# HUSRCF/JaTSR-Just-audio-transformer-super-solution

Hardware: AMD Instinct MI355X
Metric: DiT latent-frames/sec (B=28,C=1024,T=512, 50-step CFG) (higher is better)
Workload: dtype bf16; 1 GPU; v3mod2 DiT 50-step CFG=3.0 flow-matching sampling, hipGraph, B=28/GPU C=1024 T=512; B_per_gpu=28, global_batch=28, T=512, C=1024, euler_steps=50, weights=recipe (random-init, non-zero adaLN/final), parallelism=replicas x1, no collective in the loop, rccl_ranks=1

## Files before the change

### include/jat_hip.h

```cpp
#ifndef JAT_HIP_H
#define JAT_HIP_H

#include <stddef.h>
#include <stdint.h>

#ifdef __cplusplus
extern "C" {
#endif

#define JAT_OK 0
#define JAT_E_INVALID (-1)
#define JAT_E_HIP (-2)
#define JAT_E_STATE (-3)
#define JAT_E_SEQLEN (-4)

#define JAT_NORM_RMS_W 0
#define JAT_NORM_LN_NOAFFINE 1

typedef struct jat_model jat_model;
typedef struct jat_sampler jat_sampler;

typedef struct jat_config {
  int32_t input_channels;
  int32_t cond_channels;
// ... 73 lines not shown
                      float max_grad_norm, float loss_scale, int32_t step, float* grad_norm_out, void* stream);

int jat_k_norm_modulate(const float* x, const float* w, const float* shift, const float* scale,
                        int64_t mod_bstride, uint16_t* y_bf16, int32_t M, int32_t D, int32_t rows_per_batch,
                        int32_t norm_mode, void* stream);
int jat_k_gemm(const uint16_t* A, const uint16_t* W, const float* bias, void* C, int32_t M, int32_t N,
               int32_t K, int32_t epilogue, const float* gate, int64_t gate_bstride, int32_t rows_per_batch,
               int32_t variant, void* stream);
int jat_k_gemm_fold(const uint16_t* A, const uint16_t* W, const float* bias, void* C, int32_t M, int32_t N, int32_t K,
                    int32_t epilogue, const float* gate, int64_t gate_bstride, int32_t rows_per_batch, uint16_t* hi,
                    uint16_t* lo, float* part_out, const float* part_in, int32_t part_in_np, int32_t variant, void* stream);
int jat_k_gemm_splitk(const uint16_t* A, const uint16_t* W, float* parts, int32_t M, int32_t N, int32_t K, int32_t ksplit,
                      int32_t variant, void* stream);
int jat_k_qkv_attn(const uint16_t* A, const uint16_t* Wg, const float* bias, uint16_t* out, int32_t M, int32_t Hkv, int32_t K,
                   const float* rope_inv_freq, const float* part_in, int32_t part_in_np, void* stream);
int jat_k_gemm_wave_n(int32_t variant);
int jat_k_weight_grad(const uint16_t* dY, const uint16_t* X, float* dW, float* db, int32_t tokens, int32_t out, int32_t in,
                      int32_t ksplit, void* work, size_t work_bytes, void* stream);
int jat_k_attention(const uint16_t* q, const uint16_t* k, const uint16_t* vt, uint16_t* o, int32_t B,
                    int32_t N, int32_t Hq, int32_t Hkv, int32_t Npad, void* stream);
int jat_k_latent_loss(const float* pred, const float* target, const float* lr, float* dpred, float* out6,
                      int32_t rows, int32_t T, double latent_weight, double freq_weight, double ms_weight,
                      double consistency_weight, double low_freq_phase_ratio, double strict_cutoff, double soft_cutoff,
                      float loss_scale, void* work, size_t work_bytes, void* stream);
int jat_k_recon_loss(const float* pred, const float* target, float* dpred, float* loss_out, int64_t n, double eps,
                     float loss_scale, void* work, size_t work_bytes, void* stream);
int jat_k_cast_bf16(const float* in, uint16_t* out, int64_t n, void* stream);

int jat_k_attention_train(const uint16_t* q, const uint16_t* k, const uint16_t* vt, uint16_t* o, float* lse, int32_t B,
                          int32_t N, int32_t Hq, int32_t Hkv, int32_t Npad, uint64_t seed, int32_t site, float p, void* stream);
// ... 77 lines not shown
```

### jatsr-just-audio-transformer-super-solution_amd/_lib.py

```python
from __future__ import annotations

import ctypes as C
import os

_HERE = os.path.dirname(os.path.abspath(__file__))
OPERAND_DTYPE = os.environ.get("JAT_OPERAND_DTYPE", "bf16").lower()
if OPERAND_DTYPE not in ("bf16", "fp16", "float16", "bfloat16"):
    raise ValueError(f"JAT_OPERAND_DTYPE must be bf16 or fp16, got {OPERAND_DTYPE!r}")
OPERAND_DTYPE = "fp16" if OPERAND_DTYPE in ("fp16", "float16") else "bf16"
LIB_PATH = os.environ.get("JAT_LIB_PATH") or os.path.join(
    _HERE, "csrc", "libjat_hip_fp16.so" if OPERAND_DTYPE == "fp16" else "libjat_hip.so")

JAT_OK, JAT_E_INVALID, JAT_E_HIP, JAT_E_STATE, JAT_E_SEQLEN = 0, -1, -2, -3, -4
NORM_RMS_W, NORM_LN_NOAFFINE = 0, 1


class JatConfig(C.Structure):
    _fields_ = [(n, C.c_int32) for n in (
        "input_channels", "cond_channels", "patch_len", "hidden_size", "depth", "num_q_heads",
        "num_kv_heads", "bottleneck_dim", "mlp_hidden", "norm_mode")]


class JatDacConfig(C.Structure):
    _fields_ = [("latent_channels", C.c_int32), ("channels", C.c_int32), ("n_blocks", C.c_int32),
# ... 24 lines not shown
    "jat_attn_forward": (C.c_int, [_VP, _I32, _VP, _VP, _I32, _I32, _VP, _SZ, _VP]),
    "jat_time_embed": (C.c_int, [_VP, _VP, _VP, _I32, _VP, _SZ, _VP]),
    "jat_sampler_create": (C.c_int, [_VP, _I32, _I32, _I32, _F32, C.POINTER(_VP)]),
    "jat_sampler_destroy": (None, [_VP]),
    "jat_sampler_run": (C.c_int, [_VP, _VP, _VP, _VP, _I32, _VP]),
    "jat_sampler_info": (C.c_int, [_VP, _VP, _VP, _VP]),
    "jat_sampler_set_lengths": (C.c_int, [_VP, C.POINTER(_I32), _I32, _VP]),
    "jat_cfg_euler_step": (C.c_int, [_VP, _VP, _F32, _F32, _F32, _I32, _I32, _I32, _VP]),
    "jat_channel_affine": (C.c_int, [_VP, _VP, _VP, _VP, _I32, _I32, _I32, _I32, _VP]),
    "jat_crossfade_pair": (C.c_int, [_VP, _I32, _VP, _I32, _I32, _VP, _I32, _VP]),
    "jat_k_norm_modulate": (C.c_int, [_VP, _VP, _VP, _VP, _I64, _VP, _I32, _I32, _I32, _I32, _VP]),
    "jat_k_gemm": (C.c_int, [_VP, _VP, _VP, _VP, _I32, _I32, _I32, _I32, _VP, _I64, _I32, _I32, _VP]),
    "jat_k_gemm_fold": (C.c_int, [_VP, _VP, _VP, _VP, _I32, _I32, _I32, _I32, _VP, _I64, _I32, _VP, _VP, _VP, _VP, _I32, _I32, _VP]),
    "jat_k_gemm_splitk": (C.c_int, [_VP, _VP, _VP, _I32, _I32, _I32, _I32, _I32, _VP]),
    "jat_k_gemm_wave_n": (C.c_int, [_I32]),
    "jat_k_qkv_attn": (C.c_int, [_VP, _VP, _VP, _VP, _I32, _I32, _I32, _VP, _VP, _I32, _VP]),
    "jat_k_weight_grad": (C.c_int, [_VP, _VP, _VP, _VP, _I32, _I32, _I32, _I32, _VP, _SZ, _VP]),
    "jat_k_attention": (C.c_int, [_VP, _VP, _VP, _VP, _I32, _I32, _I32, _I32, _I32, _VP]),
    "jat_k_recon_loss": (C.c_int, [_VP, _VP, _VP, _VP, _I64, C.c_double, _F32, _VP, _SZ, _VP]),
    "jat_k_cast_bf16": (C.c_int, [_VP, _VP, _I64, _VP]),
    "jat_k_attention_train": (C.c_int, [_VP] * 5 + [_I32] * 5 + [C.c_uint64, _I32, _F32, _VP]),
    "jat_k_attention_bwd": (C.c_int, [_VP] * 9 + [_I32] * 5 + [C.c_uint64, _I32, _F32, _I32, _VP, _SZ, _VP]),
    "jat_k_norm_bwd": (C.c_int, [_VP, _VP, _VP, _VP, _I64, _VP, _I32, _VP, _VP, _I64, _VP] + [_I32] * 4 + [_VP, _SZ, _VP]),
    "jat_k_gate_bwd": (C.c_int, [_VP, _VP, _VP, _I64, _VP, _VP, _I64] + [_I32] * 3 + [C.c_uint64, _I32, _F32, _I32, _F32] +
                       [_VP, _SZ, _VP]),
    "jat_k_resid_gate": (C.c_int, [_VP, _VP, _VP, _I64, _VP] + [_I32] * 3 + [C.c_uint64, _I32, _F32, _I32, _F32, _VP]),
    "jat_k_gelu": (C.c_int, [_VP, _VP, _I64, C.c_uint64, _I32, _F32, _VP]),
    "jat_k_gelu_bwd": (C.c_int, [_VP, _VP, _I64, C.c_uint64, _I32, _F32, _VP]),
    "jat_k_adamw": (C.c_int, [_VP, _VP, _VP, _VP, _I64] + [_F32] * 7 + [_I32, _VP, _VP, _SZ, _VP]),
    "jat_k_small_dw": (C.c_int, [_VP, _I64, _VP, _I64, _VP, _VP] + [_I32] * 4 + [_VP]),
# ... 89 lines not shown
```

### jatsr-just-audio-transformer-super-solution_amd/csrc/elementwise.hip

```cpp
#include "jat_kernels.h"
#include "jat_gelu.h"
#include "jat_dtype.h"
#include <cstdlib>

__device__ __forceinline__ unsigned short f2bf_e(float f) { return jat_f2op(f); }
__device__ __forceinline__ uint2 pack4_e(float a, float b, float c, float d) {
  uint2 r;
  r.x = jat_pack2(a, b);
  r.y = jat_pack2(c, d);
  return r;
}
__device__ __forceinline__ float wave_sum(float v) {
#pragma unroll
  for (int o = 32; o > 0; o >>= 1) v += __shfl_xor(v, o);
  return v;
}
__device__ __forceinline__ float silu_f(float x) { return x / (1.0f + __expf(-x)); }

__global__ void __launch_bounds__(256) norm_modulate_kernel(const float* __restrict__ x, const float* __restrict__ w,
                                                            const float* __restrict__ shift,
                                                            const float* __restrict__ scale, int64_t mod_bstride,
                                                            bf16_t* __restrict__ y, int M, int D, int ntok, int mode) {
  const int lane = threadIdx.x & 63;
  const int row = blockIdx.x * 4 + (threadIdx.x >> 6);
// ... 343 lines not shown
  return hipGetLastError();
}
__global__ void gather_cast_rows_kernel(const float* __restrict__ in, int64_t in_stride, bf16_t* __restrict__ out, int rows,
                                        int cols) {
  const int i = blockIdx.x * blockDim.x + threadIdx.x;
  if (i >= rows * cols) return;
  const int r = i / cols, k = i - r * cols;
  out[(int64_t)r * cols + k] = f2bf_e(in[(int64_t)r * in_stride + k]);
}
hipError_t launch_gather_cast_rows(const float* in, int64_t in_stride, bf16_t* out, int rows, int cols, hipStream_t s) {
  const int n = rows * cols;
  hipLaunchKernelGGL(gather_cast_rows_kernel, dim3((n + 255) / 256), dim3(256), 0, s, in, in_stride, out, rows, cols);
  return hipGetLastError();
}

__global__ void __launch_bounds__(256) cfg_euler_kernel(const float* __restrict__ xp, float* __restrict__ z,
                                                        float cfg_scale, float denom, float dt, int use_cfg,
                                                        int direct, int64_t n) {
  const int64_t stride = (int64_t)gridDim.x * blockDim.x * 4;
  for (int64_t i = ((int64_t)blockIdx.x * blockDim.x + threadIdx.x) * 4; i < n; i += stride) {
    if (i + 3 < n) {
      float4 c = *(const float4*)(xp + i);
      if (use_cfg) {
        const float4 u = *(const float4*)(xp + n + i);
        c.x = u.x + cfg_scale * (c.x - u.x); c.y = u.y + cfg_scale * (c.y - u.y);
        c.z = u.z + cfg_scale * (c.z - u.z); c.w = u.w + cfg_scale * (c.w - u.w);
      }
      if (!direct) {
        const float4 zz = *(const float4*)(z + i);
        c.x = zz.x + __fdiv_rn(c.x - zz.x, denom) * dt; c.y = zz.y + __fdiv_rn(c.y - zz.y, denom) * dt;
// ... 233 lines not shown
```

### jatsr-just-audio-transformer-super-solution_amd/csrc/gemm.hip

```cpp
#include "jat_kernels.h"
#include "jat_dtype.h"

#include <type_traits>

typedef jat_opx8 bf16x8;
typedef __attribute__((ext_vector_type(4))) float f32x4;
typedef __attribute__((ext_vector_type(4))) unsigned u32x4;
typedef __attribute__((address_space(3))) void* lds_ptr_t;

template <int I, int N, class F>
__device__ __forceinline__ void static_for(F&& f) {
  if constexpr (I < N) {
    f(std::integral_constant<int, I>{});
    static_for<I + 1, N>(f);
  }
}

__device__ __forceinline__ unsigned short f2bf(float f) { return jat_f2op(f); }
__device__ __forceinline__ uint2 pack4(float a, float b, float c, float d) {
  uint2 r;
  r.x = jat_pack2(a, b);
  r.y = jat_pack2(c, d);
  return r;
}
// ... 939 lines not shown
      }
    JAT_TLX(4)
    if (m0 + q < p.M) {
#pragma unroll
      for (int h = 0; h < G; ++h) {
        bf16_t* op = (bf16_t*)p.out + (int64_t)(m0 + q) * p.ldo + (hbase + h) * 64 + fg * 4;
#pragma unroll
        for (int dt = 0; dt < 4; ++dt)
          *(uint2*)(op + dt * 16) = pack4(o[h][dt][0] * inv[h], o[h][dt][1] * inv[h], o[h][dt][2] * inv[h], o[h][dt][3] * inv[h]);
      }
    }
    JAT_TL_FLUSH()
    return;
  }

#pragma unroll
  for (int i = 0; i < TM; ++i) {
    const int m = m0 + wm * TM * 16 + i * 16 + frow;
    if (m >= p.M) continue;
    int b = 0, pos = m;
    if constexpr (EPI == EPI_RESID || EPI == EPI_QKV_ROPE || EPI == EPI_UNPATCH) {
      b = m / p.ntok;
      pos = m - b * p.ntok;
    }
    const float rstd_d = rstd_rows[i];
#pragma unroll
    for (int j = 0; j < TN; ++j) {
      const int nt = nw0 + j * 16;
      const int n = nt + fg * 4;
      f32x4 v = acc[i][j] * rstd_d;
      if constexpr (EPI == EPI_QKV_ROPE) {
        if (nt < p.D + p.kvD) {
          const int d0 = ((nt & 63) >> 1) + fg * 2;
          const float2 c = *(const float2*)(p.rope_cos + (int64_t)pos * 32 + d0);
          const float2 s = *(const float2*)(p.rope_sin + (int64_t)pos * 32 + d0);
          const float o0 = v[0] * c.x - v[1] * s.x, o1 = v[1] * c.x + v[0] * s.x;
// ... 22 lines not shown
          const float4 g = *(const float4*)(p.gate + (int64_t)b * p.gate_bstride + n);
          float4* xp = (float4*)((float*)p.out + (int64_t)m * p.ldo + n);
          float4 x = *xp;
          x.x += g.x * v[0]; x.y += g.y * v[1]; x.z += g.z * v[2]; x.w += g.w * v[3];
          *xp = x;
        } else if constexpr (EPI == EPI_UNPATCH) {
          const int c = n >> 2, t0 = pos * 4;
          float* dst = (float*)p.out + ((int64_t)b * p.C_out + c) * p.T_orig + t0;
          if ((p.T_orig & 3) == 0) {
            *(float4*)dst = float4{v[0], v[1], v[2], v[3]};
          } else {
#pragma unroll
            for (int r = 0; r < 4; ++r)
              if (t0 + r < p.T_orig) dst[r] = v[r];
          }
        }
      }
    }
  }
}

template <int WM, int WN, int TM, int TN, int EPI>
__global__ void __launch_bounds__(WM * WN * 64, 1) gemm_persist_kernel(const GemmArgs p) {
  constexpr int BM = WM * TM * 16, BN = WN * TN * 16;
  constexpr int NW = WM * WN;
  constexpr int A_BYTES = BM * 128, B_BYTES = BN * 128, STAGE = A_BYTES + B_BYTES;
  static_assert(NW == 8 && TM * TN > 20, "the row-split quadrant ping-pong of the large wave tiles");
  static_assert(EPI == EPI_BF16 || EPI == EPI_BF16_GELU, "consumer epilogues only");
  constexpr int TMa = (TM + 1) / 2, TMb = TM - TMa, TNa = (TN + 1) / 2, TNb = TN - TNa;
  constexpr int PA0 = WM * TMa * 2, PA1 = WM * TMb * 2, PB0 = WN * TNa * 2, PB1 = WN * TNb * 2;
// ... 613 lines not shown
  const int tiles = ((a.M + BM - 1) / BM) * (a.N / BN);
  if (a.ksplit > 1 && EPI != EPI_F32) return hipErrorInvalidValue;
  hipLaunchKernelGGL(kern, dim3(tiles, a.ksplit > 1 ? a.ksplit : 1), dim3((WM * WN + (PIPE == 6 ? 4 : 0)) * 64), LDS, s, a);
  return hipGetLastError();
}

template <int WM, int WN, int TM, int TN, int PIPE, int CE = 0>
static hipError_t launch_epi(const GemmArgs& a, int epi, hipStream_t s) {
  switch (epi) {
    case EPI_F32: return launch_one<WM, WN, TM, TN, PIPE, CE, EPI_F32>(a, s);
    case EPI_BF16: return launch_one<WM, WN, TM, TN, PIPE, CE, EPI_BF16>(a, s);
    case EPI_BF16_GELU: return launch_one<WM, WN, TM, TN, PIPE, CE, EPI_BF16_GELU>(a, s);
    case EPI_RESID: return launch_one<WM, WN, TM, TN, PIPE, CE, EPI_RESID>(a, s);
    case EPI_QKV_ROPE: return launch_one<WM, WN, TM, TN, PIPE, CE, EPI_QKV_ROPE>(a, s);
    case EPI_UNPATCH: return launch_one<WM, WN, TM, TN, PIPE, CE, EPI_UNPATCH>(a, s);
  }
  return hipErrorInvalidValue;
}

static const int kVariantTile[][2] = {
    {0, 0}, {0, 0}, {0, 0}, {0, 0}, {0, 0}, {0, 0}, {0, 0}, {0, 0}, {0, 0}, {0, 0},
    {128, 64},
    {0, 0}, {0, 0}, {0, 0}, {0, 0}, {0, 0}, {0, 0}, {0, 0},
    {128, 160}, {0, 0}, {128, 128}, {256, 256},
    {0, 0}, {0, 0}, {0, 0},
    {256, 160}, {256, 128},
    {64, 160}, {64, 128},
    {0, 0}, {0, 0},
    {224, 320}, {256, 160}, {256, 256}, {128, 448},
    {224, 256},
// ... 54 lines not shown
```

### jatsr-just-audio-transformer-super-solution_amd/csrc/jat_api.cpp

```cpp
#include "../../include/jat_hip.h"

#include <hip/hip_runtime.h>

#include <cmath>
#include <cstdarg>
#include <cstdio>
#include <cstdlib>
#include <cstring>
#include <string>
#include <unordered_map>
#include <vector>

#include "jat_internal.h"
#include "jat_dtype.h"

static thread_local char g_err[512] = "";
int jat_fail(int code, const char* fmt, ...) {
  va_list ap;
  va_start(ap, fmt);
  vsnprintf(g_err, sizeof(g_err), fmt, ap);
  va_end(ap);
  return code;
}

// ... 62 lines not shown
    return fail(JAT_E_INVALID, "channel counts must be positive multiples of 32");
  if (c->depth <= 0) return fail(JAT_E_INVALID, "depth must be positive");
  if (c->norm_mode != JAT_NORM_RMS_W && c->norm_mode != JAT_NORM_LN_NOAFFINE)
    return fail(JAT_E_INVALID, "unknown norm_mode");
  jat_model* m = new jat_model();
  m->cfg = *c;
  m->D = c->hidden_size; m->depth = c->depth; m->Hq = c->num_q_heads; m->Hkv = c->num_kv_heads;
  m->kvD = m->Hkv * HEAD_DIM; m->mlp = c->mlp_hidden; m->bott = c->bottleneck_dim;
  m->Cin = c->input_channels; m->Cc = c->cond_channels; m->P = 4;
  m->Kp = m->P * (m->Cin + m->Cc); m->Fout = m->P * m->Cin;
  auto env_int = [](const char* name, int dflt) { const char* v = getenv(name); return v ? atoi(v) : dflt; };
  m->sw.fuse_qkv_attn = env_int("JAT_FUSE_QKV_ATTN", 1); m->sw.qkv_split = env_int("JAT_QKV_SPLIT", 1);
  m->sw.fuse_finish = env_int("JAT_FUSE_FINISH", 1); m->sw.fold_norm = env_int("JAT_FOLD_NORM", 1);
  m->sw.split_patch = env_int("JAT_SPLIT_PATCH", 1);
  m->sw.fold_cap_mb = env_int("JAT_FOLD_CAP_MB", 0); m->sw.patch_split = env_int("JAT_PATCH_SPLIT", 1);
  if (const char* v = getenv("JAT_GEMM_VARIANT"))
    for (int i = 0; i < 5; ++i) m->variants[i] = atoi(v);
  if (const char* v = getenv("JAT_GEMM_VARIANTS")) {
    int x[5];
    if (sscanf(v, "%d,%d,%d,%d,%d", &x[0], &x[1], &x[2], &x[3], &x[4]) == 5)
      for (int i = 0; i < 5; ++i) m->variants[i] = x[i];
  }
  *out = m;
  return JAT_OK;
}

extern "C" int jat_model_set_switch(jat_model* m, const char* name, int32_t value) {
  if (!m || !name) return fail(JAT_E_INVALID, "null argument");
  const std::string n(name);
  int* slot = n == "fuse_qkv_attn" ? &m->sw.fuse_qkv_attn : n == "qkv_split" ? &m->sw.qkv_split : n == "fuse_finish" ? &m->sw.fuse_finish
            : n == "fold_norm" ? &m->sw.fold_norm : n == "split_patch" ? &m->sw.split_patch
            : n == "fold_cap_mb" ? &m->sw.fold_cap_mb : n == "patch_split" ? &m->sw.patch_split : nullptr;
  if (!slot) return fail(JAT_E_INVALID, "unknown switch '%s'", name);
  *slot = value;
  return JAT_OK;
}

extern "C" void jat_model_destroy(jat_model* m) {
  if (!m) return;
  for (hipEvent_t e : m->prof.ev) (void)hipEventDestroy(e);
  if (m->blob) (void)hipFree(m->blob);
  delete m;
}

extern "C" int jat_model_load_weights(jat_model* m, const jat_tensor_ref* named, int32_t n, void* stream_) {
  if (!m || !named) return fail(JAT_E_INVALID, "null argument");
  return jat_pack_weights(m, named, n, (hipStream_t)stream_, true);
// ... 237 lines not shown
  KCHK(launch_linear_f32(w.e_sin, m->te_w1, m->te_b1, w.t_h, nullptr, B, m->D, m->D, 1, s));
  KCHK(launch_linear_f32(w.t_h, m->te_w2, m->te_b2, w.t_emb, w.t_silu, B, m->D, m->D, 0, s));
  return JAT_OK;
}
static int adaln_path(const jat_model* m, const bf16_t* t_silu, float* mod, int B, int l0, int nl, hipStream_t s) {
  GemmArgs e{};
  e.out = mod; e.ldo = (int64_t)nl * 6 * m->D; e.bias = m->bada + (int64_t)l0 * 6 * m->D; e.ntok = 1;
  return gemm(m, G_OTHER, t_silu, m->D, m->wada + (int64_t)l0 * 6 * m->D * m->D, m->D, B, nl * 6 * m->D, m->D, EPI_F32, e, s);
}

struct Fold {
  const bf16_t *wqkv_g, *wqkv_i, *w1, *wfinal;
  const float *bq_g, *bq_i, *bf;
};

static int resid_split(const jat_model* m, const Workspace& w, int site, int M, int K, bool folding, int* variant = nullptr) {
  if (variant) *variant = -1;
  if (!w.kpart || folding || K < 1024 || m->variants[site] >= 0) return 1;
  auto slices = [&](int v, int cap) {
    int bm, bn;
    gemm_variant_tile(v, &bm, &bn);
    const int tiles = ((M + bm - 1) / bm) * (m->D / bn), slots = (v == 18 || v == 20 || v == 27 || v == 28) ? 512 : 256;
    int split = slots / tiles < cap ? slots / tiles : cap;
    while (split > 1 && ((K / 64) % split != 0 || K / split < 256)) --split;
    return split > 1 ? split : 1;
  };
  if (M <= kSplitMaxRows) return slices((K >= 4096 || M >= 1536) ? 20 : pick_variant(M, m->D), kSplitMax);
  static const int kpair_split = getenv("JAT_KPAIR_SPLIT") ? atoi(getenv("JAT_KPAIR_SPLIT")) : 1;
  if (kpair_split && variant && M % 224 == 0 && m->D % 160 == 0) {
    const int tiles = (M / 224) * (m->D / 160);
// ... 104 lines not shown
        KCHK(launch_splitk_resid_norm(w.kpart, split, (int64_t)M * D, L.b2, mod_l + 5 * D, bstride, w.x, next->w, next->shift,
                                      next->scale, bstride, w.xn, M, D, ntok, m->cfg.norm_mode, s));
        if (next_done) *next_done = true;
      } else {
        KCHK(launch_splitk_resid_finish(w.kpart, split, (int64_t)M * D, L.b2, mod_l + 5 * D, bstride, ntok, w.x, M, D, s));
      }
    } else {
      JCHK(gemm(m, G_FC2, w.hm, m->mlp, L.w2, m->mlp, M, D, m->mlp, EPI_RESID, e, s));
    }
  }
  return JAT_OK;
}

static int forward_impl(const jat_model* m, const Workspace& w, const float* x_t, int B_src, const float* x_cond,
                        int cond_zero_from, const float* t, const float* mod, int64_t mod_bstride, float* x_pred,
                        int B, int T, hipStream_t s, const Fold* f = nullptr, const float* pc = nullptr) {
  const int ntok = (T + 3) / 4, M = B * ntok, D = m->D;
  if (!mod) {
    JCHK(time_path(m, w, t, B, s));
    JCHK(adaln_path(m, w.t_silu, w.mod, B, 0, m->depth, s));
    mod = w.mod;
    mod_bstride = (int64_t)m->depth * 6 * D;
  }
  if (t) HIPCHK(hipMemsetAsync(w.vt, 0, w.vt_bytes, s));
  auto patch_split = [&](int rows, int K) {
    if (!m->sw.patch_split || m->variants[G_OTHER] >= 0 || m->bott % 128 != 0) return 1;
    const int tiles = ((rows + 63) / 64) * (m->bott / 128);
    if (tiles > 128 && K < 8192) return 1;
    int split = 512 / tiles, cap = m->mlp / (2 * m->bott);
    if (cap > 4) cap = 4;
    if (split > cap) split = cap;
    while (split > 1 && ((K / 64) % split != 0 || K / split < 1024)) --split;
    return split > 1 ? split : 1;
  };
  if (pc) {
    const int Mh = M / 2, Kz = m->P * m->Cin;
    KCHK(launch_patchify(x_t, nullptr, w.a_patch, B_src, B_src, B_src, m->Cin, 0, T, ntok, s, w.tvalid));
    const int ps = patch_split(Mh, Kz);
    if (ps > 1) {
      GemmArgs e{};
      e.out = w.hm; e.ldo = m->bott; e.ntok = ntok; e.ksplit = ps; e.split_stride = (int64_t)Mh * m->bott;
      JCHK(gemm(m, G_OTHER, w.a_patch, Kz, m->pe_w1, m->Kp, Mh, m->bott, Kz, EPI_F32, e, s));
      KCHK(launch_splitk_gelu_finish((const float*)w.hm, ps, (int64_t)Mh * m->bott, m->pe_b1, pc, Mh, w.h_patch, m->bott, Mh, m->bott, s));
    } else {
      GemmArgs e{};
      e.out = w.h_patch; e.ldo = m->bott; e.bias = m->pe_b1; e.ntok = ntok; e.dual_add = pc; e.dual_rows = Mh;
      JCHK(gemm(m, G_OTHER, w.a_patch, Kz, m->pe_w1, m->Kp, Mh, m->bott, Kz, EPI_BF16_GELU, e, s));
    }
  } else {
    KCHK(launch_patchify(x_t, x_cond, w.a_patch, B, B_src, cond_zero_from, m->Cin, m->Cc, T, ntok, s, w.tvalid));
    const int ps = patch_split(M, m->Kp);
    if (ps > 1) {
// ... 9 lines not shown
  }
  {
    GemmArgs e{};
    e.out = w.x; e.ldo = D; e.bias = m->pe_b2; e.ntok = ntok;
    if (f) { e.fold_out = w.xn; e.fold_lo = w.xlo; e.fold_part = w.part; }
    JCHK(gemm(m, G_OTHER, w.h_patch, m->bott, m->pe_w2, m->bott, M, D, m->bott, EPI_F32, e, s));
  }
  bool xn_ready = false;
  for (int l = 0; l < m->depth; ++l) {
    const float* mod_n = mod + (int64_t)(l + 1) * 6 * D;
    const NextNorm nn = l + 1 < m->depth ? NextNorm{m->layers[l + 1].norm1, mod_n + 0 * D, mod_n + 1 * D}
                                         : NextNorm{m->final_norm, nullptr, nullptr};
    bool done = false;
    JCHK(run_block(m, w, l, B, ntok, mod + (int64_t)l * 6 * D, mod_bstride, s, f, xn_ready, &nn, &done));
    xn_ready = done;
  }
  if (!f && !xn_ready) KCHK(launch_norm_modulate(w.x, m->final_norm, nullptr, nullptr, 0, w.xn, M, D, ntok, m->cfg.norm_mode, s));
  {
    GemmArgs e{};
    e.out = x_pred; e.bias = m->bfinal; e.ntok = ntok; e.C_out = m->Cin; e.T_orig = T;
    if (f) e.rs_part = w.part;
    JCHK(gemm(m, G_OTHER, w.xn, D, f ? f->wfinal : m->wfinal, D, M, m->Fout, D, EPI_UNPATCH, e, s));
  }
  return JAT_OK;
}

static int check_ready(const jat_model* m, int B, int ntok, void* ws, size_t ws_bytes, Workspace* w) {
  if (!m) return fail(JAT_E_INVALID, "null model");
  if (!m->loaded) return fail(JAT_E_STATE, "weights not loaded");
  if (B <= 0 || ntok <= 0) return fail(JAT_E_INVALID, "B and T must be positive");
// ... 71 lines not shown

struct jat_sampler {
  jat_model* m;
  int B, T, steps, Bf;
  float cfg_scale;
  bool use_cfg;
  std::vector<float> ts;
  char* blob = nullptr;
  float *z, *lr, *xpred, *mod_table, *ts_dev;
  std::shared_ptr<FoldTable> fold;
  bool fused_attn = false;
  float* pc = nullptr;
  int* lens_dev = nullptr;
  int* frames_dev = nullptr;
  bool folded = false;
  void* ws;
  size_t ws_bytes;
  Workspace w;
  hipStream_t cap_stream = nullptr;
  hipGraph_t graph = nullptr;
  hipGraphExec_t exec = nullptr;
};

static void linspace01(int n, std::vector<float>& out) {
  out.resize(n);
  const float step = 1.0f / (float)(n - 1);
  for (int i = 0; i < n; ++i)
    out[i] = i < n / 2 ? (float)((double)step * i) : (float)(1.0 - (double)step * (n - 1 - i));
}

// ... 11 lines not shown
  jat_model* m = sp->m;
  const int64_t n_half = (int64_t)sp->B * m->Cin * sp->T;
  const int64_t row = (int64_t)m->depth * 6 * m->D;
  for (int i = 0; i < sp->steps; ++i) {
    const float t_curr = sp->ts[i], dt = sp->ts[i + 1] - sp->ts[i];
    Fold f{};
    if (sp->folded) {
      const FoldTable& ft = *sp->fold;
      const int64_t Nqkv = m->D + 2 * m->kvD, dl = m->depth;
      if (sp->fused_attn) { f.wqkv_g = ft.qkv_g + (int64_t)i * dl * Nqkv * m->D; f.bq_g = ft.bq_g + (int64_t)i * dl * Nqkv; }
      else { f.wqkv_i = ft.qkv_i + (int64_t)i * dl * Nqkv * m->D; f.bq_i = ft.bq_i + (int64_t)i * dl * Nqkv; }
      f.w1 = ft.w1 + (int64_t)i * dl * m->mlp * m->D;
      f.bf = ft.bf + (int64_t)i * dl * m->mlp;
      f.wfinal = ft.wfinal;
    }
    JCHK(forward_impl(m, sp->w, sp->z, sp->B, sp->lr, sp->B, nullptr, sp->mod_table + i * row, 0, sp->xpred, sp->Bf,
                      sp->T, s, sp->folded ? &f : nullptr, sp->pc));
    KCHK(launch_cfg_euler(sp->xpred, sp->z, sp->cfg_scale, t_curr, dt, sp->use_cfg ? 1 : 0, n_half, s));
  }
  return JAT_OK;
}

static int fold_alloc(FoldTable& ft, void** p, size_t bytes) {
  if (hipMalloc(p, bytes) != hipSuccess) { (void)hipGetLastError(); return fail(JAT_E_HIP, "hipMalloc(%zu) for the folded weights", bytes); }
  ft.allocs.push_back(*p);
  return JAT_OK;
}
static int build_fold_table_impl(jat_model* m, FoldTable& ft, int steps, const float* mod, bool group_major, bf16_t* sh_bf16,
                                 hipStream_t s, bool need_w1, bool need_qkv);
static int build_fold_table(jat_model* m, FoldTable& ft, int steps, const float* mod, bool group_major, bf16_t* sh_bf16,
                            hipStream_t s) {
  const bool need_w1 = ft.w1 == nullptr;
  const bool need_qkv = group_major ? ft.qkv_g == nullptr : ft.qkv_i == nullptr;
// ... 138 lines not shown
      const size_t need = (size_t)steps * m->depth * ((Nq + m->mlp) * m->D * 2 + (Nq + m->mlp) * 4) + (size_t)m->Fout * m->D * 2;
      const bool over_cap = m->sw.fold_cap_mb > 0 && need > (size_t)m->sw.fold_cap_mb * 1048576;
      std::shared_ptr<FoldTable>& slot = m->fold_cache[steps];
      if (!slot) slot = std::make_shared<FoldTable>();
      if (over_cap || build_fold_table(m, *slot, steps, sp->mod_table, sp->fused_attn, sh_bf16, s) != JAT_OK) {
        (void)hipStreamSynchronize(s);
        if (!slot->w1 && !slot->qkv_g && !slot->qkv_i) m->fold_cache.erase(steps);
        sp->folded = false;
      } else {
        sp->fold = slot;
      }
    }
    if (hipStreamSynchronize(s) != hipSuccess) return bail(fail(JAT_E_HIP, "sync after table build"));
  }
  sp->w = carve(m, sp->Bf, ntok, (char*)sp->ws);
  if (hipMemsetAsync(sp->w.vt, 0, sp->w.vt_bytes, s) != hipSuccess) return bail(fail(JAT_E_HIP, "memset vt"));
  {
    std::vector<int> full((size_t)sp->Bf, ntok), fullT((size_t)B, T);
    if (hipMemcpyAsync(sp->lens_dev, full.data(), full.size() * 4, hipMemcpyHostToDevice, s) != hipSuccess ||
        hipMemcpyAsync(sp->frames_dev, fullT.data(), fullT.size() * 4, hipMemcpyHostToDevice, s) != hipSuccess ||
        hipStreamSynchronize(s) != hipSuccess)
      return bail(fail(JAT_E_HIP, "lengths upload"));
    if (!sp->fused_attn) { sp->w.lens = sp->lens_dev; sp->w.tvalid = sp->frames_dev; }
  }

  if (hipMemsetAsync(sp->z, 0, lat, s) != hipSuccess || hipMemsetAsync(sp->lr, 0, lat, s) != hipSuccess)
    return bail(fail(JAT_E_HIP, "memset"));
  {
    const int saved = sp->steps;
    sp->steps = 1;
// ... 132 lines not shown
  KCHK(launch_gemm(a, epilogue, variant, (hipStream_t)stream));
  return JAT_OK;
}
extern "C" int jat_k_qkv_attn(const uint16_t* A, const uint16_t* Wg, const float* bias, uint16_t* out, int32_t M, int32_t Hkv,
                              int32_t K, const float* rope_inv_freq, const float* part_in, int32_t part_in_np, void* stream) {
  if (!A || !Wg || !out || !rope_inv_freq || M <= 0 || M % 128 != 0 || K % 64 != 0) return fail(JAT_E_INVALID, "bad argument");
  GemmArgs a{};
  a.A = A; a.lda = K; a.W = Wg; a.ldw = K; a.M = M; a.N = Hkv * 448; a.K = K;
  a.out = out; a.ldo = (int64_t)Hkv * 320; a.ntok = 128; a.rope_inv_freq = rope_inv_freq; a.bias = bias;
  a.attn_scale_log2e = 0.125f * 1.4426950408889634f;
  a.rs_part = part_in; a.rs_np = part_in_np;
  if (const char* d = getenv("JAT_GEMM_TIMELINE")) a.dbg_out = (unsigned long long*)strtoull(d, nullptr, 0);
  KCHK(launch_qkv_attn(a, (hipStream_t)stream));
  return JAT_OK;
}
extern "C" int jat_k_weight_grad(const uint16_t* dY, const uint16_t* X, float* dW, float* db, int32_t tokens, int32_t out,
                                 int32_t in, int32_t ksplit, void* work, size_t work_bytes, void* stream) {
  if (!gemm_tn_supports(out, in)) return fail(JAT_E_INVALID, "out and in must be multiples of 128");
  if (tokens <= 0) return fail(JAT_E_INVALID, "tokens must be positive");
  if (ksplit == 0) ksplit = gemm_tn_ksplit(out, in, tokens);
  if (ksplit < 1 || ksplit > (tokens + 63) / 64) return fail(JAT_E_INVALID, "bad ksplit");
  const int64_t area = (int64_t)out * in;
  const size_t part_f = ksplit > 1 ? (size_t)ksplit * area : 0, col_f = db ? (size_t)colsum_slices(tokens) * out : 0;
  const size_t need = 256 + (part_f + col_f) * 4;
  if (!work || work_bytes < need) return fail(JAT_E_INVALID, "work needs %zu bytes", need);
  hipStream_t s = (hipStream_t)stream;
  HIPCHK(hipMemsetAsync(work, 0, 256, s));
  float* part = (float*)((char*)work + 256);
  KCHK(launch_gemm_tn(dY, out, X, in, ksplit > 1 ? part : dW, in, out, in, tokens, ksplit, area, work, s));
  if (ksplit > 1) KCHK(launch_sum_partials(part, ksplit, area, dW, area, s));
// ... 58 lines not shown
```

### jatsr-just-audio-transformer-super-solution_amd/csrc/jat_internal.h

```cpp
#pragma once
#include "../../include/jat_hip.h"

#include <hip/hip_runtime.h>

#include <map>
#include <memory>
#include <string>
#include <vector>

#include "jat_kernels.h"

int jat_fail(int code, const char* fmt, ...);
#define fail jat_fail
#define HIPCHK(expr)                                                                                   \
  do {                                                                                                 \
    hipError_t e__ = (expr);                                                                           \
    if (e__ != hipSuccess) return fail(JAT_E_HIP, "%s failed: %s (%s:%d)", #expr, hipGetErrorString(e__), \
                                       __FILE__, __LINE__);                                            \
  } while (0)
#define JCHK(expr)            \
  do {                        \
    int r__ = (expr);         \
    if (r__ != JAT_OK) return r__; \
  } while (0)
// ... 19 lines not shown
  bf16_t *qkv_g = nullptr, *qkv_i = nullptr;
  bf16_t *w1 = nullptr, *wfinal = nullptr;
  float *bq_g = nullptr, *bq_i = nullptr, *bf = nullptr;
  std::vector<void*> allocs;
  ~FoldTable() { for (void* p : allocs) (void)hipFree(p); }
};

struct jat_switches {
  int fuse_qkv_attn = 1;
  int qkv_split = 1;
  int fuse_finish = 1;
  int fold_norm = 1;
  int split_patch = 1;
  int fold_cap_mb = 0;
  int patch_split = 1;
};
struct GemmProf {
  int site = -1, n = 0, variant = -1;
  double flops = 0.0;
  hipStream_t stream = nullptr;
  std::vector<hipEvent_t> ev;
};

struct jat_model {
  jat_config cfg;
  jat_switches sw;
  mutable GemmProf prof;
  int D, depth, Hq, Hkv, kvD, mlp, bott, Cin, Cc, P, Kp, Fout;
  bool loaded = false;
  char* blob = nullptr;
// ... 17 lines not shown
```

### jatsr-just-audio-transformer-super-solution_amd/csrc/jat_kernels.h

```cpp
#pragma once
#include <hip/hip_runtime.h>
#include <stdint.h>

#include "jat_rng.h"

typedef uint16_t bf16_t;

enum GemmEpi : int {
  EPI_F32 = 0,
  EPI_BF16 = 1,
  EPI_BF16_GELU = 2,
  EPI_RESID = 3,
  EPI_QKV_ROPE = 4,
  EPI_QKV_ATTN = 6,
  EPI_UNPATCH = 5,
};

struct GemmArgs {
  const bf16_t* A;
  const bf16_t* W;
  int64_t lda, ldw;
  int M, N, K;
  void* out;
  int64_t ldo;
  const float* bias;
  const float* gate;
  int64_t gate_bstride;
  int ntok;
  bf16_t* k_out;
  bf16_t* vt_out;
// ... 3 lines not shown
  const float* rope_inv_freq;
  int C_out, T_orig;
  bf16_t* fold_out;
  bf16_t* fold_lo;
  float* fold_part;
  int fold_np;
  const float* rs_part;
  int rs_np;
  float attn_scale_log2e;
  const float* dual_add;
  int dual_rows;
  unsigned long long* dbg_out;
  int ksplit;
  int64_t split_stride;
  int variant_hint;
};

hipError_t launch_gemm(const GemmArgs& a, int epi, int variant, hipStream_t s);
int gemm_num_variants();
bool gemm_variant_exists(int variant);
hipError_t launch_qkv_attn(const GemmArgs& a, hipStream_t s);
void gemm_variant_tile(int variant, int* bm, int* bn);
int gemm_variant_wave_n(int variant);
bool gemm_variant_coalesced(int variant);

struct AttnArgs {
  const bf16_t* q;
  const bf16_t* k;
  const bf16_t* vt;
  bf16_t* o;
// ... 21 lines not shown
                                    bf16_t* q, bf16_t* k, bf16_t* vt, int M, int D, int kvD, int ntok, int npad, hipStream_t s);
bool splitk_resid_norm_supported(int D);
hipError_t launch_splitk_resid_norm(const float* part, int nsplit, int64_t stride, const float* bias, const float* gate,
                                    int64_t gate_bstride, float* x, const float* w, const float* shift, const float* scale,
                                    int64_t mod_bstride, bf16_t* y, int M, int D, int ntok, int mode, hipStream_t s);
hipError_t launch_splitk_resid_finish(const float* part, int nsplit, int64_t stride, const float* bias, const float* gate,
                                      int64_t gate_bstride, int ntok, float* x, int M, int N, hipStream_t s);
hipError_t launch_silu_bf16(const float* in, bf16_t* out, int64_t n, hipStream_t s);
hipError_t launch_cast_bf16(const float* in, bf16_t* out, int64_t n, hipStream_t s);
hipError_t launch_cast_bf16_rope_rows(const float* in, bf16_t* out, int rows, int cols, hipStream_t s);
hipError_t launch_fold_weight(const float* in, const float* w, const float* scale, bf16_t* out, int rows, int cols, int rope,
                              hipStream_t s);
hipError_t launch_fold_scale(const float* w, const float* scale, int64_t in_stride, float* out, int64_t out_stride,
                             int rows, int cols, hipStream_t s);
hipError_t launch_gather_cast_rows(const float* in, int64_t in_stride, bf16_t* out, int rows, int cols, hipStream_t s);
hipError_t launch_cfg_euler(const float* xp, float* z, float cfg_scale, float t, float dt, int use_cfg,
                            int64_t n_per_half, hipStream_t s);
hipError_t launch_channel_affine(const float* in, const float* mean, const float* std, float* out, int B,
                                 int C, int T, int inverse, hipStream_t s);
hipError_t launch_crossfade_pair(const float* prev, int Tp, const float* cur, int Tc, int overlap,
                                 float* out, int rows, hipStream_t s);

hipError_t launch_sum_partials(const float* part, int nsplit, int64_t stride, float* out, int64_t n, hipStream_t s);
hipError_t launch_transpose_bf16(const bf16_t* in, int64_t ld_in, int M, int C, bf16_t* out, int Mpad, hipStream_t s);
hipError_t launch_rowsum_bf16(const bf16_t* x, int64_t ld, int R, int n, float* out, hipStream_t s);
bool gemm_tn_supports(int M, int N);
int gemm_tn_ksplit(int M, int N, int K);
hipError_t launch_gemm_tn(const bf16_t* dY, int64_t ldy, const bf16_t* X, int64_t ldx, float* dW, int64_t ldo, int M, int N, int K,
                          int ksplit, int64_t split_stride, const void* zeros, hipStream_t s);
int colsum_slices(int R);
// ... 40 lines not shown
```

Measured before the change: 40610 latent-frames/s.

## Fuse CFG combine, final projection, Euler update and re-patchify into sampler tail

Adds a sampler tail path. It first combines the conditional and unconditional normalized hidden states, using each row's folded rstd and the CFG weights, before the final projection. The final GEMM then runs on half the rows, and its epilogue applies the Euler update to z and writes the next step's bf16 patch input directly. This removes the full-batch final GEMM, the separate cfg_euler kernel, the x_pred round-trip and the per-step patchify launch. It relies on CFG being linear through the final projection, and adds bf16 rounding of the combined activations.

```diff
diff --git a/include/jat_hip.h b/include/jat_hip.h
--- a/include/jat_hip.h
+++ b/include/jat_hip.h
@@ -111,6 +111,10 @@
                       int32_t variant, void* stream);
 int jat_k_qkv_attn(const uint16_t* A, const uint16_t* Wg, const float* bias, uint16_t* out, int32_t M, int32_t Hkv, int32_t K,
                    const float* rope_inv_freq, const float* part_in, int32_t part_in_np, void* stream);
+int jat_k_unpatch_euler(const uint16_t* A, const uint16_t* W, const float* bias, float* z, uint16_t* patch_out,
+                        const int32_t* frames, int32_t B, int32_t C, int32_t T, int32_t K, float t, float dt, int32_t variant,
+                        void* stream);
+int jat_k_patchify(const float* x, uint16_t* out, const int32_t* frames, int32_t B, int32_t C, int32_t T, void* stream);
 int jat_k_gemm_wave_n(int32_t variant);
 int jat_k_weight_grad(const uint16_t* dY, const uint16_t* X, float* dW, float* db, int32_t tokens, int32_t out, int32_t in,
                       int32_t ksplit, void* work, size_t work_bytes, void* stream);
diff --git a/jatsr-just-audio-transformer-super-solution_amd/_lib.py b/jatsr-just-audio-transformer-super-solution_amd/_lib.py
--- a/jatsr-just-audio-transformer-super-solution_amd/_lib.py
+++ b/jatsr-just-audio-transformer-super-solution_amd/_lib.py
@@ -62,6 +62,8 @@
     "jat_k_gemm_fold": (C.c_int, [_VP, _VP, _VP, _VP, _I32, _I32, _I32, _I32, _VP, _I64, _I32, _VP, _VP, _VP, _VP, _I32, _I32, _VP]),
     "jat_k_gemm_splitk": (C.c_int, [_VP, _VP, _VP, _I32, _I32, _I32, _I32, _I32, _VP]),
     "jat_k_gemm_wave_n": (C.c_int, [_I32]),
+    "jat_k_unpatch_euler": (C.c_int, [_VP, _VP, _VP, _VP, _VP, _VP, _I32, _I32, _I32, _I32, _F32, _F32, _I32, _VP]),
+    "jat_k_patchify": (C.c_int, [_VP, _VP, _VP, _I32, _I32, _I32, _VP]),
     "jat_k_qkv_attn": (C.c_int, [_VP, _VP, _VP, _VP, _I32, _I32, _I32, _VP, _VP, _I32, _VP]),
     "jat_k_weight_grad": (C.c_int, [_VP, _VP, _VP, _VP, _I32, _I32, _I32, _I32, _VP, _SZ, _VP]),
     "jat_k_attention": (C.c_int, [_VP, _VP, _VP, _VP, _I32, _I32, _I32, _I32, _I32, _VP]),
diff --git a/jatsr-just-audio-transformer-super-solution_amd/csrc/elementwise.hip b/jatsr-just-audio-transformer-super-solution_amd/csrc/elementwise.hip
--- a/jatsr-just-audio-transformer-super-solution_amd/csrc/elementwise.hip
+++ b/jatsr-just-audio-transformer-super-solution_amd/csrc/elementwise.hip
@@ -381,6 +381,45 @@
   return hipGetLastError();
 }
 
+__device__ __forceinline__ float fold_rstd_e(const float* __restrict__ part, int np, float invk) {
+  float g[4];
+#pragma unroll
+  for (int j = 0; j < 4; ++j) {
+    g[j] = 0.f;
+    if (4 * j < np) {
+      const f32x4_e q = *(const f32x4_e*)(part + 4 * j);
+      g[j] = (q[0] + q[1]) + (q[2] + q[3]);
+    }
+  }
+  const float sq = np == 4 ? g[0] : np == 8 ? g[0] + g[1] : (g[0] + g[1]) + (g[2] + g[3]);
+  return rsqrtf(sq * invk + 1e-6f);
+}
+__global__ void __launch_bounds__(256) cfg_combine_kernel(const bf16_t* __restrict__ hi, const float* __restrict__ part, int np,
+                                                          float cfg_scale, bf16_t* __restrict__ out, int Mh, int D) {
+  const int64_t i = (int64_t)blockIdx.x * 256 + threadIdx.x;
+  const int per_row = D / 8;
+  if (i >= (int64_t)Mh * per_row) return;
+  const int row = (int)(i / per_row), c = (int)(i % per_row) * 8;
+  const float invk = 1.0f / (float)D;
+  const float wc = cfg_scale * fold_rstd_e(part + (int64_t)row * np, np, invk);
+  const float wu = (1.0f - cfg_scale) * fold_rstd_e(part + (int64_t)(row + Mh) * np, np, invk);
+  const uint4 a = *(const uint4*)(hi + (int64_t)row * D + c);
+  const uint4 b = *(const uint4*)(hi + (int64_t)(row + Mh) * D + c);
+  const unsigned av[4] = {a.x, a.y, a.z, a.w}, bv[4] = {b.x, b.y, b.z, b.w};
+  unsigned o[4];
+#pragma unroll
+  for (int k = 0; k < 4; ++k)
+    o[k] = jat_pack2(wc * jat_lo2f(av[k]) + wu * jat_lo2f(bv[k]), wc * jat_hi2f(av[k]) + wu * jat_hi2f(bv[k]));
+  *(uint4*)(out + (int64_t)row * D + c) = uint4{o[0], o[1], o[2], o[3]};
+}
+hipError_t launch_cfg_combine(const bf16_t* hi, const float* part, int np, float cfg_scale, bf16_t* out, int Mh, int D,
+                              hipStream_t s) {
+  if (D % 8 != 0 || Mh <= 0 || (np != 4 && np != 8 && np != 16)) return hipErrorInvalidValue;
+  const int64_t n = (int64_t)Mh * (D / 8);
+  hipLaunchKernelGGL(cfg_combine_kernel, dim3((unsigned)((n + 255) / 256)), dim3(256), 0, s, hi, part, np, cfg_scale, out, Mh, D);
+  return hipGetLastError();
+}
+
 __global__ void __launch_bounds__(256) cfg_euler_kernel(const float* __restrict__ xp, float* __restrict__ z,
                                                         float cfg_scale, float denom, float dt, int use_cfg,
                                                         int direct, int64_t n) {
diff --git a/jatsr-just-audio-transformer-super-solution_amd/csrc/gemm.hip b/jatsr-just-audio-transformer-super-solution_amd/csrc/gemm.hip
--- a/jatsr-just-audio-transformer-super-solution_amd/csrc/gemm.hip
+++ b/jatsr-just-audio-transformer-super-solution_amd/csrc/gemm.hip
@@ -977,12 +977,56 @@
     return;
   }
 
+  if constexpr (EPI == EPI_UNPATCH_EULER) {
+    if ((p.T_orig & 3) == 0) {
+      float4 zb[2][TN];
+      int tvb[2];
+      auto load = [&](int i, int k) {
+        const int m = min(m0 + wm * TM * 16 + i * 16 + frow, p.M - 1);
+        const int b = m / p.ntok, pos = m - b * p.ntok;
+        tvb[k] = p.tvalid ? min(p.tvalid[b], p.T_orig) : p.T_orig;
+#pragma unroll
+        for (int j = 0; j < TN; ++j) {
+          const int c = (nw0 + j * 16 + fg * 4) >> 2;
+          zb[k][j] = *(const float4*)((const float*)p.out + ((int64_t)b * p.C_out + c) * p.T_orig + pos * 4);
+        }
+      };
+      load(0, 0);
+      static_for<0, TM>([&](auto I) {
+        constexpr int i = decltype(I)::value, k = i & 1;
+        if constexpr (i + 1 < TM) load(i + 1, k ^ 1);
+        const int m = m0 + wm * TM * 16 + i * 16 + frow;
+        if (m < p.M) {
+          const int b = m / p.ntok, pos = m - b * p.ntok, t0 = pos * 4;
+#pragma unroll
+          for (int j = 0; j < TN; ++j) {
+            const int n = nw0 + j * 16 + fg * 4, c = n >> 2;
+            f32x4 v = acc[i][j] * rstd_rows[i];
+            if (p.bias) {
+              const float4 bb = *(const float4*)(p.bias + n);
+              v[0] += bb.x; v[1] += bb.y; v[2] += bb.z; v[3] += bb.w;
+            }
+            const float zo[4] = {zb[k][j].x, zb[k][j].y, zb[k][j].z, zb[k][j].w};
+            float zn[4];
+#pragma unroll
+            for (int r = 0; r < 4; ++r) zn[r] = p.euler_direct ? v[r] : zo[r] + __fdiv_rn(v[r] - zo[r], p.euler_denom) * p.euler_dt;
+            *(float4*)((float*)p.out + ((int64_t)b * p.C_out + c) * p.T_orig + t0) = float4{zn[0], zn[1], zn[2], zn[3]};
+#pragma unroll
+            for (int r = 0; r < 4; ++r) zn[r] = t0 + r < tvb[k] ? zn[r] : 0.f;
+            *(uint2*)(p.patch_out + (int64_t)m * p.ldo + n) = pack4(zn[0], zn[1], zn[2], zn[3]);
+          }
+        }
+      });
+      return;
+    }
+  }
+
 #pragma unroll
   for (int i = 0; i < TM; ++i) {
     const int m = m0 + wm * TM * 16 + i * 16 + frow;
     if (m >= p.M) continue;
     int b = 0, pos = m;
-    if constexpr (EPI == EPI_RESID || EPI == EPI_QKV_ROPE || EPI == EPI_UNPATCH) {
+    if constexpr (EPI == EPI_RESID || EPI == EPI_QKV_ROPE || EPI == EPI_UNPATCH || EPI == EPI_UNPATCH_EULER) {
       b = m / p.ntok;
       pos = m - b * p.ntok;
     }
@@ -1035,6 +1079,31 @@
             for (int r = 0; r < 4; ++r)
               if (t0 + r < p.T_orig) dst[r] = v[r];
           }
+        } else if constexpr (EPI == EPI_UNPATCH_EULER) {
+          const int c = n >> 2, t0 = pos * 4;
+          float* zp = (float*)p.out + ((int64_t)b * p.C_out + c) * p.T_orig + t0;
+          const int tv = p.tvalid ? min(p.tvalid[b], p.T_orig) : p.T_orig;
+          float zn[4];
+          if ((p.T_orig & 3) == 0) {
+            const float4 zz = *(const float4*)zp;
+            const float zo[4] = {zz.x, zz.y, zz.z, zz.w};
+#pragma unroll
+            for (int r = 0; r < 4; ++r) zn[r] = p.euler_direct ? v[r] : zo[r] + __fdiv_rn(v[r] - zo[r], p.euler_denom) * p.euler_dt;
+            *(float4*)zp = float4{zn[0], zn[1], zn[2], zn[3]};
+          } else {
+#pragma unroll
+            for (int r = 0; r < 4; ++r) {
+              zn[r] = 0.f;
+              if (t0 + r < p.T_orig) {
+                const float zo = zp[r];
+                zn[r] = p.euler_direct ? v[r] : zo + __fdiv_rn(v[r] - zo, p.euler_denom) * p.euler_dt;
+                zp[r] = zn[r];
+              }
+            }
+          }
+#pragma unroll
+          for (int r = 0; r < 4; ++r) zn[r] = t0 + r < tv ? zn[r] : 0.f;
+          *(uint2*)(p.patch_out + (int64_t)m * p.ldo + n) = pack4(zn[0], zn[1], zn[2], zn[3]);
         }
       }
     }
@@ -1678,6 +1747,7 @@
     case EPI_RESID: return launch_one<WM, WN, TM, TN, PIPE, CE, EPI_RESID>(a, s);
     case EPI_QKV_ROPE: return launch_one<WM, WN, TM, TN, PIPE, CE, EPI_QKV_ROPE>(a, s);
     case EPI_UNPATCH: return launch_one<WM, WN, TM, TN, PIPE, CE, EPI_UNPATCH>(a, s);
+    case EPI_UNPATCH_EULER: return launch_one<WM, WN, TM, TN, PIPE, CE, EPI_UNPATCH_EULER>(a, s);
   }
   return hipErrorInvalidValue;
 }
diff --git a/jatsr-just-audio-transformer-super-solution_amd/csrc/jat_api.cpp b/jatsr-just-audio-transformer-super-solution_amd/csrc/jat_api.cpp
--- a/jatsr-just-audio-transformer-super-solution_amd/csrc/jat_api.cpp
+++ b/jatsr-just-audio-transformer-super-solution_amd/csrc/jat_api.cpp
@@ -100,6 +100,7 @@
   m->sw.fuse_finish = env_int("JAT_FUSE_FINISH", 1); m->sw.fold_norm = env_int("JAT_FOLD_NORM", 1);
   m->sw.split_patch = env_int("JAT_SPLIT_PATCH", 1);
   m->sw.fold_cap_mb = env_int("JAT_FOLD_CAP_MB", 0); m->sw.patch_split = env_int("JAT_PATCH_SPLIT", 1);
+  m->sw.cfg_tail = env_int("JAT_CFG_TAIL", 1);
   if (const char* v = getenv("JAT_GEMM_VARIANT"))
     for (int i = 0; i < 5; ++i) m->variants[i] = atoi(v);
   if (const char* v = getenv("JAT_GEMM_VARIANTS")) {
@@ -116,7 +117,8 @@
   const std::string n(name);
   int* slot = n == "fuse_qkv_attn" ? &m->sw.fuse_qkv_attn : n == "qkv_split" ? &m->sw.qkv_split : n == "fuse_finish" ? &m->sw.fuse_finish
             : n == "fold_norm" ? &m->sw.fold_norm : n == "split_patch" ? &m->sw.split_patch
-            : n == "fold_cap_mb" ? &m->sw.fold_cap_mb : n == "patch_split" ? &m->sw.patch_split : nullptr;
+            : n == "fold_cap_mb" ? &m->sw.fold_cap_mb : n == "patch_split" ? &m->sw.patch_split
+            : n == "cfg_tail" ? &m->sw.cfg_tail : nullptr;
   if (!slot) return fail(JAT_E_INVALID, "unknown switch '%s'", name);
   *slot = value;
   return JAT_OK;
@@ -384,6 +386,13 @@
   const float *bq_g, *bq_i, *bf;
 };
 
+struct Tail {
+  float* z;
+  float cfg_scale, denom, dt;
+  int direct;
+  bool first;
+};
+
 static int resid_split(const jat_model* m, const Workspace& w, int site, int M, int K, bool folding, int* variant = nullptr) {
   if (variant) *variant = -1;
   if (!w.kpart || folding || K < 1024 || m->variants[site] >= 0) return 1;
@@ -518,7 +527,8 @@
 
 static int forward_impl(const jat_model* m, const Workspace& w, const float* x_t, int B_src, const float* x_cond,
                         int cond_zero_from, const float* t, const float* mod, int64_t mod_bstride, float* x_pred,
-                        int B, int T, hipStream_t s, const Fold* f = nullptr, const float* pc = nullptr) {
+                        int B, int T, hipStream_t s, const Fold* f = nullptr, const float* pc = nullptr,
+                        const Tail* tail = nullptr) {
   const int ntok = (T + 3) / 4, M = B * ntok, D = m->D;
   if (!mod) {
     JCHK(time_path(m, w, t, B, s));
@@ -539,7 +549,7 @@
   };
   if (pc) {
     const int Mh = M / 2, Kz = m->P * m->Cin;
-    KCHK(launch_patchify(x_t, nullptr, w.a_patch, B_src, B_src, B_src, m->Cin, 0, T, ntok, s, w.tvalid));
+    if (!tail || tail->first) KCHK(launch_patchify(x_t, nullptr, w.a_patch, B_src, B_src, B_src, m->Cin, 0, T, ntok, s, w.tvalid));
     const int ps = patch_split(Mh, Kz);
     if (ps > 1) {
       GemmArgs e{};
@@ -579,6 +589,16 @@
     bool done = false;
     JCHK(run_block(m, w, l, B, ntok, mod + (int64_t)l * 6 * D, mod_bstride, s, f, xn_ready, &nn, &done));
     xn_ready = done;
+  }
+  if (tail) {
+    const int Mh = M / 2;
+    KCHK(launch_cfg_combine(w.xn, w.part, m->last_fold_np, tail->cfg_scale, w.ao, Mh, D, s));
+    GemmArgs e{};
+    e.out = tail->z; e.bias = m->bfinal; e.ntok = ntok; e.C_out = m->Cin; e.T_orig = T;
+    e.patch_out = w.a_patch; e.ldo = m->Fout; e.tvalid = w.tvalid;
+    e.euler_denom = tail->denom; e.euler_dt = tail->dt; e.euler_direct = tail->direct;
+    JCHK(gemm(m, G_OTHER, w.ao, D, f->wfinal, D, Mh, m->Fout, D, EPI_UNPATCH_EULER, e, s));
+    return JAT_OK;
   }
   if (!f && !xn_ready) KCHK(launch_norm_modulate(w.x, m->final_norm, nullptr, nullptr, 0, w.xn, M, D, ntok, m->cfg.norm_mode, s));
   {
@@ -680,6 +700,7 @@
   int* lens_dev = nullptr;
   int* frames_dev = nullptr;
   bool folded = false;
+  bool cfg_tail = false;
   void* ws;
   size_t ws_bytes;
   Workspace w;
@@ -721,9 +742,10 @@
       f.bf = ft.bf + (int64_t)i * dl * m->mlp;
       f.wfinal = ft.wfinal;
     }
+    const Tail tl{sp->z, sp->cfg_scale, 1.0f - t_curr + 1e-5f, dt, !(t_curr < 0.999f) ? 1 : 0, i == 0};
     JCHK(forward_impl(m, sp->w, sp->z, sp->B, sp->lr, sp->B, nullptr, sp->mod_table + i * row, 0, sp->xpred, sp->Bf,
-                      sp->T, s, sp->folded ? &f : nullptr, sp->pc));
-    KCHK(launch_cfg_euler(sp->xpred, sp->z, sp->cfg_scale, t_curr, dt, sp->use_cfg ? 1 : 0, n_half, s));
+                      sp->T, s, sp->folded ? &f : nullptr, sp->pc, sp->cfg_tail ? &tl : nullptr));
+    if (!sp->cfg_tail) KCHK(launch_cfg_euler(sp->xpred, sp->z, sp->cfg_scale, t_curr, dt, sp->use_cfg ? 1 : 0, n_half, s));
   }
   return JAT_OK;
 }
@@ -892,6 +914,7 @@
     if (hipStreamSynchronize(s) != hipSuccess) return bail(fail(JAT_E_HIP, "sync after table build"));
   }
   sp->w = carve(m, sp->Bf, ntok, (char*)sp->ws);
+  sp->cfg_tail = m->sw.cfg_tail && sp->use_cfg && sp->folded && sp->pc;
   if (hipMemsetAsync(sp->w.vt, 0, sp->w.vt_bytes, s) != hipSuccess) return bail(fail(JAT_E_HIP, "memset vt"));
   {
     std::vector<int> full((size_t)sp->Bf, ntok), fullT((size_t)B, T);
@@ -1054,6 +1077,27 @@
   KCHK(launch_qkv_attn(a, (hipStream_t)stream));
   return JAT_OK;
 }
+extern "C" int jat_k_unpatch_euler(const uint16_t* A, const uint16_t* W, const float* bias, float* z, uint16_t* patch_out,
+                                   const int32_t* frames, int32_t B, int32_t C, int32_t T, int32_t K, float t, float dt,
+                                   int32_t variant, void* stream) {
+  if (!A || !W || !z || !patch_out || B <= 0 || C <= 0 || T <= 0 || C % 32 != 0 || K <= 0 || K % 64 != 0)
+    return fail(JAT_E_INVALID, "bad argument");
+  const int ntok = (T + 3) / 4;
+  if (variant == 0) variant = pick_variant(B * ntok, 4 * C);
+  if (!gemm_variant_exists(variant)) return fail(JAT_E_INVALID, "unknown GEMM variant %d", variant);
+  GemmArgs a{};
+  a.A = A; a.lda = K; a.W = W; a.ldw = K; a.M = B * ntok; a.N = 4 * C; a.K = K;
+  a.out = z; a.bias = bias; a.ntok = ntok; a.C_out = C; a.T_orig = T;
+  a.patch_out = patch_out; a.ldo = 4 * C; a.tvalid = frames;
+  a.euler_denom = 1.0f - t + 1e-5f; a.euler_dt = dt; a.euler_direct = !(t < 0.999f) ? 1 : 0;
+  KCHK(launch_gemm(a, EPI_UNPATCH_EULER, variant, (hipStream_t)stream));
+  return JAT_OK;
+}
+extern "C" int jat_k_patchify(const float* x, uint16_t* out, const int32_t* frames, int32_t B, int32_t C, int32_t T, void* stream) {
+  if (!x || !out || B <= 0 || T <= 0 || C <= 0 || C % 32 != 0) return fail(JAT_E_INVALID, "bad argument");
+  KCHK(launch_patchify(x, nullptr, out, B, B, B, C, 0, T, (T + 3) / 4, (hipStream_t)stream, frames));
+  return JAT_OK;
+}
 extern "C" int jat_k_weight_grad(const uint16_t* dY, const uint16_t* X, float* dW, float* db, int32_t tokens, int32_t out,
                                  int32_t in, int32_t ksplit, void* work, size_t work_bytes, void* stream) {
   if (!gemm_tn_supports(out, in)) return fail(JAT_E_INVALID, "out and in must be multiples of 128");
diff --git a/jatsr-just-audio-transformer-super-solution_amd/csrc/jat_internal.h b/jatsr-just-audio-transformer-super-solution_amd/csrc/jat_internal.h
--- a/jatsr-just-audio-transformer-super-solution_amd/csrc/jat_internal.h
+++ b/jatsr-just-audio-transformer-super-solution_amd/csrc/jat_internal.h
@@ -57,6 +57,7 @@
   int split_patch = 1;
   int fold_cap_mb = 0;
   int patch_split = 1;
+  int cfg_tail = 1;
 };
 struct GemmProf {
   int site = -1, n = 0, variant = -1;
diff --git a/jatsr-just-audio-transformer-super-solution_amd/csrc/jat_kernels.h b/jatsr-just-audio-transformer-super-solution_amd/csrc/jat_kernels.h
--- a/jatsr-just-audio-transformer-super-solution_amd/csrc/jat_kernels.h
+++ b/jatsr-just-audio-transformer-super-solution_amd/csrc/jat_kernels.h
@@ -14,6 +14,7 @@
   EPI_QKV_ROPE = 4,
   EPI_QKV_ATTN = 6,
   EPI_UNPATCH = 5,
+  EPI_UNPATCH_EULER = 7,
 };
 
 struct GemmArgs {
@@ -47,6 +48,10 @@
   int ksplit;
   int64_t split_stride;
   int variant_hint;
+  bf16_t* patch_out;
+  const int* tvalid;
+  float euler_denom, euler_dt;
+  int euler_direct;
 };
 
 hipError_t launch_gemm(const GemmArgs& a, int epi, int variant, hipStream_t s);
@@ -98,6 +103,8 @@
 hipError_t launch_fold_scale(const float* w, const float* scale, int64_t in_stride, float* out, int64_t out_stride,
                              int rows, int cols, hipStream_t s);
 hipError_t launch_gather_cast_rows(const float* in, int64_t in_stride, bf16_t* out, int rows, int cols, hipStream_t s);
+hipError_t launch_cfg_combine(const bf16_t* hi, const float* part, int np, float cfg_scale, bf16_t* out, int Mh, int D,
+                              hipStream_t s);
 hipError_t launch_cfg_euler(const float* xp, float* z, float cfg_scale, float t, float dt, int use_cfg,
                             int64_t n_per_half, hipStream_t s);
 hipError_t launch_channel_affine(const float* in, const float* mean, const float* std, float* out, int B,
```

Result: faster. 41160 latent-frames/s, median of 6 (+1.4%).
